# lab-emi/OpenDPD

Hardware: AMD Instinct MI355X
Metric: iq_samples_per_sec_train (higher is better)
Workload: dtype f32

## Files before the change

### opendpd_amd/csrc/capi.hip

```cpp
#include <dlfcn.h>

#include <mutex>
#include <set>
#include <utility>

#include "odpd_host.h"
#include "odpd_xchg.h"

using namespace odpd;

namespace {
enum Family { FAM_NONE = 0, FAM_GRU, FAM_LSTM, FAM_DELTA, FAM_JANET, FAM_TCNN, FAM_QAT, FAM_GMP, FAM_RVTDCNN, FAM_DVR, FAM_BOJ, FAM_APN, FAM_MCL, FAM_GRU2, FAM_QCELL };
inline Family family_of(int bb);
inline Family family_of(const odpd_model_t* m) {
    if (m->flags & ODPD_FLAG_QUANT_CELL) return FAM_QCELL;
    if (m->flags & ODPD_FLAG_TWO_LAYERS) return FAM_GRU2;
    if (m->bits_w > 0 && (m->backbone == ODPD_QGRU || m->backbone == ODPD_QGRU_AMP1 || m->backbone == ODPD_GRU || m->backbone == ODPD_DGRU ||
                          m->backbone == ODPD_TRES_DELTAGRU))
        return FAM_QAT;
    return family_of((int)m->backbone);
}
inline Family family_of(int bb) {
    switch (bb) {
    case ODPD_GRU: case ODPD_DGRU: case ODPD_QGRU: case ODPD_QGRU_AMP1: return FAM_GRU;
// ... 709 lines not shown
extern "C" int odpd_sweep_fwd_supported(const odpd_model_t* m, int B, int T) {
    return model_ok(m) && gru_family_model(m) && gru_sweep_eval_ok(m, B, T) ? 1 : 0;
}
extern "C" int odpd_sweep_s16_supported(const odpd_model_t* m) {
    return model_ok(m) && gru_family_model(m) && gru_s16_sweep_ok(m) ? 1 : 0;
}
extern "C" int64_t odpd_sweep_partial_rows(const odpd_model_t* m, int B, int T, int flags) {
    if (!model_ok(m) || B <= 0 || T <= 0 || !gru_family_model(m)) return ODPD_EUNSUPPORTED;
    if (flags & ODPD_SWEEP_S16) return gru_s16_sweep_ok(m) ? gru_s16_rows(m, B) : (int64_t)ODPD_EUNSUPPORTED;
    return gru_sweep_train_ok(m, B, T) ? gru_sweep_train_rows(m, B, T) : (int64_t)ODPD_EUNSUPPORTED;
}
extern "C" int64_t odpd_sweep_workspace_floats(const odpd_model_t* m, int B, int T, int flags) {
    if (!model_ok(m) || B <= 0 || T <= 0) return ODPD_EINVAL;
    if (init_state(m) || quant_cell(m)) return ODPD_EUNSUPPORTED;
    if (!(flags & ODPD_SWEEP_S16)) return 0;
    return odpd_sweep_s16_supported(m) ? gru_s16_ckpt_floats(m, B, T) : (int64_t)ODPD_EUNSUPPORTED;
}
extern "C" int odpd_train_epoch_sweep(void* stream, const odpd_model_t* m, int K, const odpd_sweep_run_t* runs, int loss_kind, const odpd_frames_t* fr,
                                      int batch, int64_t first_step, double beta1, double beta2, double eps, double weight_decay, double max_norm,
                                      int flags, void* scratch) {
    if (!model_ok(m) || K <= 0 || !runs || !epoch_frames_ok(fr, batch, false) || first_step <= 0 || !scratch) return ODPD_EINVAL;
    if (!sweep_runs_ok(K, runs, [](int) { return true; })) return ODPD_EINVAL;
    const int T = fr->frame_length;
    const bool s16 = (flags & ODPD_SWEEP_S16) != 0;
    if (!gru_family_model(m) || !frames_format_ok(m, fr)) return ODPD_EUNSUPPORTED;
    if (s16) {
        if (!gru_s16_sweep_ok(m)) return ODPD_EUNSUPPORTED;
        for (int k = 0; k < K; ++k)
            if (!runs[k].workspace) return ODPD_EINVAL;
    } else if (!epoch_shapes_served(fr, batch, 0, 1, [&](int B) { return gru_sweep_train_ok(m, B, T); })) {
        return ODPD_EUNSUPPORTED;
// ... 78 lines not shown
```

### opendpd_amd/csrc/gru_family.hip

```cpp
#include <algorithm>

#include "odpd_gru.h"

namespace odpd {

template <int R, int F, bool DG>
struct GruW {
    float wih[3][F];
    float b_r, b_z, b_in, b_hn;
    float wout[2], bout[2];
    float bhid;
    float woutf[2];
};

template <int R, int F, bool DG>
__device__ __forceinline__ void load_gru_w(GruW<R, F, DG>& w, const float* pl, const GruLayout& L, int row, int col) {
    const int H = L.H, o = 16 * row + col;
    const bool vo = o < H;
#pragma unroll
    for (int g = 0; g < 3; ++g)
#pragma unroll
        for (int i = 0; i < F; ++i) w.wih[g][i] = vo ? pl[L.o_w_ih + (g * H + o) * F + i] : 0.0f;
    w.b_r = vo ? pl[L.o_b_ih + o] + pl[L.o_b_hh + o] : 0.0f;
    w.b_z = vo ? pl[L.o_b_ih + H + o] + pl[L.o_b_hh + H + o] : 0.0f;
// ... 1330 lines not shown
        p.fwd_eval = eval || (knobs_free && B <= 8 && T >= 256) ? KS_EVAL : big;
        const bool bwd_gp = R == 1 && !s16 && knobs_free && (long)B <= (long)device_cus() * gp_blocks_per_cu(P, R, DG, T, false);
        p.bwd_w = bwd_gp ? KS_GP : big;
        p.bwd_dx = p.bwd_wdx = big;
        p.rot_rows = bwd_shape(R, ng).grid;
        p.bwd_rows = s16n ? gru_s16n_rows(m, B) : s16 ? gru_s16_bwd_rows(m, B) : bwd_gp ? std::max(gp_grid(P, R, DG, B, T), p.rot_rows) : p.rot_rows;
    }
    if (parts & GRU_PLAN_FUSED) {
        const int rot_grid = big == KS_ROT ? train_shape(P, R, DG, ng, T, nullptr).grid : 0;
        const bool too_long = R == 1 && rot_grid <= 0;
        if (big != KS_ROT) p.fused = big;
        else if (too_long) p.fused = KS_S16;
        else p.fused = gp_batch_fits(B, gp_blocks_per_cu(P, R, DG, T, false), 1) ? KS_GP : KS_ROT;
        switch (p.fused) {
        case KS_S16X: case KS_S16N: p.fused_rows = gru_s16n_rows(m, B); p.ws_floats = s16n_floats(); break;
        case KS_S16: p.fused_rows = gru_s16_rows(m, B); p.ws_floats = gru_s16_ckpt_floats(m, B, T); break;
        case KS_GP: p.fused_rows = gp_grid(P, R, DG, B, T); break;
        default: p.fused_rows = rot_grid > 0 ? rot_grid : ODPD_EUNSUPPORTED;
        }
    }
    if (parts & GRU_PLAN_LOSSDX) {
        const bool no_gain = R == 2 && !DG && m->hidden > 24 && tn.gp_max_batch < 0, knob_bars = tn.gp_max_batch >= 0 && B > tn.gp_max_batch;
        const int fz_grid = big == KS_ROT && !no_gain && !knob_bars ? gp_fz_grid(P, R, DG, B, T) : 0;
        p.lossdx = s16n ? (gru_s16x_ok(m) ? KS_S16X : KS_S16N) : s16 ? KS_S16 : fz_grid > 0 ? KS_GP : KS_ROT;
        switch (p.lossdx) {
        case KS_S16X: case KS_S16N: p.loss_rows = gru_s16n_rows(m, B); break;
        case KS_S16: p.loss_rows = gru_s16_rows(m, B); break;
        case KS_GP: p.loss_rows = fz_grid; break;
        default: {
            const int grid = train_shape(P, R, DG, ng, T, nullptr, true).grid;
            p.loss_rows = grid > 0 ? grid : ODPD_EUNSUPPORTED;
// ... 8 lines not shown
```

### opendpd_amd/csrc/gru_s16.hip

```cpp
#include "odpd_s16.h"

namespace odpd {

constexpr int kS16Groups = 15;
constexpr int kS16GroupsDx = 20;
template <int FM, bool DG, bool PACK = false>
__device__ __forceinline__ float4 s16_table_entry(const float* pl, const GruLayout& L, int grp, int m, int q) {
    const int H = L.H, OW = DG ? H + 6 : H;
    float v[4] = {0.f, 0.f, 0.f, 0.f};
#pragma unroll
    for (int e = 0; e < 4; ++e) {
        const int k = 4 * q + e;
        const bool mk = m < H && k < H;
        if (grp < 3) {
            v[e] = mk ? pl[L.o_w_hh + (grp * H + m) * H + k] * (grp < 2 ? kNegLog2e : 1.0f) : 0.0f;
            if (PACK && grp < 2 && k >= 13) v[e] = kNegLog2e * s16_wih_slot<FM, DG>(pl, L, grp, 1, m, k - 13);
        }
        else if (grp == 3) v[e] = kNegLog2e * s16_wih_slot<FM, DG>(pl, L, e >> 1, e & 1, m, q);
        else if (grp == 4) v[e] = e < 2 ? s16_wih_slot<FM, DG>(pl, L, 2, e, m, q) : 0.0f;
        else if (grp == 5) v[e] = k < H ? pl[L.o_b_hh + 2 * H + k] : 0.0f;
        else if (grp < 9) v[e] = mk ? pl[L.o_w_hh + ((grp - 6) * H + k) * H + m] : 0.0f;
        else if (grp == 9) v[e] = (DG && mk) ? pl[L.o_w_hid + m * H + k] : 0.0f;
        else if (grp == 10) v[e] = (DG && mk) ? pl[L.o_w_hid + k * H + m] : 0.0f;
        else if (grp == 11) v[e] = (DG && k < H) ? pl[L.o_b_hid + k] : 0.0f;
        else if (grp < 14) v[e] = k < H ? pl[L.o_w_out + (grp - 12) * OW + k] : 0.0f;
        else if (grp == 14) v[e] = s16_woutf_slot<FM, DG>(pl, L, e >> 1, e & 1, q);
        else if (grp < 18) v[e] = (m < S16Cfg<FM>::F && k < H) ? pl[L.o_w_ih + ((grp - 15) * H + k) * S16Cfg<FM>::F + m] : 0.0f;
        else v[e] = (DG && k < S16Cfg<FM>::F) ? pl[L.o_w_out + (grp - 18) * OW + H + k] : 0.0f;
    }
    return make_float4(v[0], v[1], v[2], v[3]);
}
template <int FM, bool DG, bool PACK = false>
__device__ __forceinline__ void s16_fill_table(float* tab, const float* pl, const GruLayout& L, int lane, int wave, int nwb,
                                               int ngroups = kS16Groups) {
    float4* t4 = reinterpret_cast<float4*>(tab);
    for (int grp = wave; grp < ngroups; grp += nwb)
        if (DG || (grp < 9 || grp > 11)) t4[grp * 64 + lane] = s16_table_entry<FM, DG, PACK>(pl, L, grp, lane & 15, lane >> 4);
    __syncthreads();
}

template <int FM>
struct S16Fw {
    float whh[3][4];
    float wih[3][2];
    f32x4 bhn;
};
template <int FM, bool DG>
struct S16Bw {
    float whhT[3][4];
    float whid[4], whidT[4];
    f32x4 bhid;
    f32x4 wout[2];
    float woutf[2][2];
};
// ... 67 lines not shown
        const f32x4 z4 = {0.f, 0.f, 0.f, 0.f};
#pragma unroll
        for (int g = 0; g < 3; ++g) { thh[g] = z4; tih[g] = z4; }
        thid = z4; db_hn = z4; db_hid = z4; dwout[0] = z4; dwout[1] = z4;
        dwf[0][0] = dwf[0][1] = dwf[1][0] = dwf[1][1] = 0.f;
#pragma unroll
        for (int j = 0; j < 4; ++j) vr[j] = vz[j] = 0.f;
    }
};
#ifdef ODPD_NO_PACKGRAD
constexpr bool s16_packgrad(bool pack, bool nw) { return false; }
#else
constexpr bool s16_packgrad(bool pack, bool nw) { return pack && nw; }
#endif

template <int FM, bool DG, bool FUSED, bool NW, bool DX, bool FULL, bool PACK = false>
__device__ __forceinline__ void s16_block(const SeqArgs& a, TabPtr tl, const float (&oh)[4], S16Grad<DG>& G,
                                          const float2* xs, const float2* ts, float2* dxs, float* tiles, int n, int q, int tloc,
                                          int nstep, bool valid, bool last_blk, f32x4 h, f32x4& dh, float (&hTn)[4],
                                          float& loss_acc) {
    constexpr int NCH = S16Cfg<FM>::NCH, S = kCkptStride;
    f32x4 hp_s[S], r_s[S], z_s[S], n_s[S], g_s[S];
    float fs_s[S][NCH];
    {
        S16Fw<FM> wf;
        s16_load_fw<FM>(wf, tl);
#pragma unroll
        for (int st = 0; st < S; ++st) {
            if (FULL || st < nstep) {
                const float2 xv = xs[n * kChunkPad + tloc + st];
                hp_s[st] = h;
                if constexpr (PACK) {
                    float pk[3];
                    s16_slots_pk<FM>(xv.x, xv.y, oh, fs_s[st], pk);
                    s16_cell_fwd<FM, true>(wf, fs_s[st], h, r_s[st], z_s[st], n_s[st], g_s[st], pk);
                } else {
// ... 13 lines not shown
        TabPtr tx = opaque(tl);
#pragma unroll
        for (int g = 0; g < 3; ++g) {
            const float4 v = tab_ld(tx, (15 + g) * 64);
            wihT[g][0] = v.x; wihT[g][1] = v.y; wihT[g][2] = v.z; wihT[g][3] = v.w;
        }
        wfD[0] = as_f32x4(tab_ld(tx, 18 * 64));
        wfD[1] = as_f32x4(tab_ld(tx, 19 * 64));
    }
    if (NW && DG && last_blk) {
        wave_lds_fence();
        tile_put(t_h, n, q, h);
        wave_lds_fence();
        tile_get(t_h, n, q, hTn);
    }
    const S16Loss lossc = s16_loss_setup(a.loss_kind == ODPD_LOSS_L2, valid ? a.inv_count : 0.0f, valid && q == 0);
#pragma unroll
    for (int st = S - 1; st >= 0; --st) {
        if (FULL || st < nstep) {
            __builtin_amdgcn_sched_barrier(0);
            const f32x4 hp = hp_s[st], r = r_s[st], z = z_s[st], nn = n_s[st], gh = g_s[st];
            f32x4 act, hid;
            const f32x4 ht = fma4(z, sub4(hp, nn), nn);
            if constexpr (DG) {
                hid = w.bhid;
#pragma unroll
                for (int c = 0; c < 4; ++c) hid = mfma4(w.whid[c], ht[c], hid);
                ODPD_EACH4 act[i] = relu_(hid[i]);
            } else {
                act = ht;
            }
// ... 1 lines not shown
            float dy0 = tv.x, dy1 = tv.y;
            if constexpr (FUSED) {
                float p0 = 0.0f, p1 = 0.0f;
#pragma unroll
                for (int c = 0; c < NCH; ++c) {
                    p0 = __builtin_fmaf(w.woutf[0][c], fs_s[st][c], p0);
                    p1 = __builtin_fmaf(w.woutf[1][c], fs_s[st][c], p1);
                }
#pragma unroll
                for (int e = 0; e < 4; ++e) {
                    p0 = __builtin_fmaf(w.wout[0][e], act[e], p0);
                    p1 = __builtin_fmaf(w.wout[1][e], act[e], p1);
                }
                const float y0 = quad_sum(p0), y1 = quad_sum(p1);
                const float d0 = y0 - tv.x, d1 = y1 - tv.y;
                s16_loss(lossc, d0, d1, dy0, dy1, loss_acc);
            }
            if constexpr (NW) {
#pragma unroll
                for (int c = 0; c < NCH; ++c) {
                    if (c < 2) {
                        G.dwf[0][c] = __builtin_fmaf(dy0, fs_s[st][c], G.dwf[0][c]);
                        G.dwf[1][c] = __builtin_fmaf(dy1, fs_s[st][c], G.dwf[1][c]);
                    }
                }
                G.dwout[0] = fma4(splat4(dy0), act, G.dwout[0]);
                G.dwout[1] = fma4(splat4(dy1), act, G.dwout[1]);
            }
            f32x4 dht, dhid;
            const f32x4 dact = fma4(splat4(dy0), w.wout[0], mul4(w.wout[1], splat4(dy1)));
            if constexpr (DG) {
// ... 163 lines not shown
        for (int c = 0; c < NCH; ++c) {
            const int k = 4 * c + q;
            const float v = row_sum16(G.dwf[cc][c < 2 ? c : 0]);
            if (n == 0) {
                if (DG && k < F) prow[L.o_w_out + cc * OW + H + k] = v;
                else if (k == F) prow[L.o_b_out + cc] = v;
            }
        }
    const float lp = row_sum16(loss_acc);
    if (n == 0 && q == 0) {
        prow[L.P] = lp;
        prow[L.P + 1] = 0.f; prow[L.P + 2] = 0.f; prow[L.P + 3] = 0.f;
    }
}

template <int FM, bool DG, int OCC, bool PACK, bool NW = true, bool DX = false>
__device__ __forceinline__ void gru16_train_body(const SeqArgs& a, const int bid, const int nbl) {
    constexpr int F = S16Cfg<FM>::F, NCH = S16Cfg<FM>::NCH, S = kCkptStride;
    constexpr int kGroups = DX ? kS16GroupsDx : kS16Groups;
    constexpr int kWave = (DX ? 3 : 2) * 2 * 16 * kChunkPad + (NW ? kS16Tiles * kTileFloats : 0) + kStageRowFloats;
    static_assert(NCH <= 2, "operand tables and dwf accumulators are sized for two K-chunks");
    extern __shared__ __attribute__((aligned(16))) float smem[];
    const int lane = threadIdx.x & 63, wave = threadIdx.x >> 6, nwb = blockDim.x >> 6;
    const int n = lane & 15, q = lane >> 4;
    const GruLayout L = gru_layout(a.H, F, DG);
    float* pl = smem;
    stage_params(pl, a.params, L.P);
    float* tab = smem + pad4(L.P);
    s16_fill_table<FM, DG, PACK>(tab, pl, L, lane, wave, nwb, kGroups);
    TabPtr tl = to_tab(reinterpret_cast<const float4*>(tab) + lane);
    float oh[4];
#pragma unroll
    for (int e = 0; e < 4; ++e) oh[e] = q == e ? 1.0f : 0.0f;
    float* wbase = tab + s16_tab_floats(kGroups) + (size_t)wave * kWave;
    float2* xs = reinterpret_cast<float2*>(wbase);
    float2* ts = xs + 16 * kChunkPad;
    float2* dxs = DX ? ts + 16 * kChunkPad : nullptr;
    float* tiles = reinterpret_cast<float*>(ts + (DX ? 2 : 1) * 16 * kChunkPad);
    unsigned long long* rows = reinterpret_cast<unsigned long long*>(wbase + kWave - kStageRowFloats);
    const bool bf16 = a.frames_bf16 != 0;
    const float2 kFillX = make_float2(0.5f, 0.5f), kFillT = make_float2(0.0f, 0.0f);
    if constexpr (NW)
        for (int i = lane; i < kTileFloats; i += 64) tiles[6 * kTileFloats + i] = 0.0f;
    S16Grad<DG> G;
    G.zero();
    float loss_acc = 0.0f;
    const int nwaves = nbl * nwb;
    for (int grp = bid * nwb + wave; grp < a.ngroups; grp += nwaves) {
        const int b0 = grp * 16;
        const bool valid = b0 + n < a.B;
        float4* ck = reinterpret_cast<float4*>(a.ckpt) + (size_t)grp * a.nck * 64 + lane;
        wave_lds_fence();
        stage_rows(rows, b0, a.B, a.T, lane, a.frame_idx, a.frame_stride);
        wave_lds_fence();
        {
            S16Fw<FM> w;
            s16_load_fw<FM>(w, tl);
            f32x4 h = {0.f, 0.f, 0.f, 0.f};
            for (int t0 = 0; t0 < a.T; t0 += kChunk) {
                const int len = min(kChunk, a.T - t0);
                StagedChunk<1> xc;
                stage_issue<1>(xc, {a.x}, rows, b0, a.B, t0, len, lane, {kFillX}, bf16);
                wave_lds_fence();
                stage_commit<1>(xc, {xs}, b0, a.B, len, lane, bf16);
                wave_lds_fence();
                int tt = 0;
                for (; tt + S <= len; tt += S) {
#pragma unroll
                    for (int i = 0; i < S; ++i) {
                        const float2 xv = xs[n * kChunkPad + tt + i];
                        float fs[NCH];
                        f32x4 r, z, nn, g;
                        if constexpr (PACK) {
                            float pk[3];
                            s16_slots_pk<FM>(xv.x, xv.y, oh, fs, pk);
                            s16_cell_fwd<FM, true>(w, fs, h, r, z, nn, g, pk);
                        } else {
                            s16_slots<FM>(xv.x, xv.y, oh, fs);
                            s16_cell_fwd<FM>(w, fs, h, r, z, nn, g);
                        }
                    }
                    const int t1 = t0 + tt + S;
                    if (t1 < a.T) ck[(size_t)(t1 / S) * 64] = make_float4(h[0], h[1], h[2], h[3]);
                }
                for (; tt < len; ++tt) {
                    const float2 xv = xs[n * kChunkPad + tt];
                    float fs[NCH];
                    f32x4 r, z, nn, g;
                    if constexpr (PACK) {
                        float pk[3];
                        s16_slots_pk<FM>(xv.x, xv.y, oh, fs, pk);
                        s16_cell_fwd<FM, true>(w, fs, h, r, z, nn, g, pk);
                    } else {
                        s16_slots<FM>(xv.x, xv.y, oh, fs);
                        s16_cell_fwd<FM>(w, fs, h, r, z, nn, g);
                    }
                }
            }
        }
        __builtin_amdgcn_fence(__ATOMIC_SEQ_CST, "workgroup");
        f32x4 dh = {0.f, 0.f, 0.f, 0.f};
        float hTn[4] = {0.f, 0.f, 0.f, 0.f};
        int cur_chunk = -1;
        float4 h0n = a.nck > 1 ? ck[(size_t)(a.nck - 1) * 64] : make_float4(0.f, 0.f, 0.f, 0.f);
        for (int blk = a.nck - 1; blk >= 0; --blk) {
            const int tb = blk * S, nstep = min(S, a.T - tb);
            const int chunk = tb / kChunk, t0 = chunk * kChunk;
            const f32x4 h0 = {h0n.x, h0n.y, h0n.z, h0n.w};
            h0n = blk > 1 ? ck[(size_t)(blk - 1) * 64] : make_float4(0.f, 0.f, 0.f, 0.f);
            if (chunk != cur_chunk) {
                if constexpr (DX) {
                    if (cur_chunk >= 0) {
                        const int pt0 = cur_chunk * kChunk;
                        wave_lds_fence();
                        stage_out<16>(dxs, a.dx, b0, a.B, a.T, pt0, min(kChunk, a.T - pt0), lane);
                    }
                }
                const int len = min(kChunk, a.T - t0);
                StagedChunk<2> xt;
                stage_issue<2>(xt, {a.x, a.target}, rows, b0, a.B, t0, len, lane, {kFillX, kFillT}, bf16);
                wave_lds_fence();
                stage_commit<2>(xt, {xs, ts}, b0, a.B, len, lane, bf16);
                wave_lds_fence();
                cur_chunk = chunk;
            }
            if (nstep == S)
                s16_block<FM, DG, true, NW, DX, true, PACK>(a, tl, oh, G, xs, ts, dxs, tiles, n, q, tb - t0, nstep, valid, blk == a.nck - 1, h0, dh, hTn, loss_acc);
            else
                s16_block<FM, DG, true, NW, DX, false, PACK>(a, tl, oh, G, xs, ts, dxs, tiles, n, q, tb - t0, nstep, valid, blk == a.nck - 1, h0, dh, hTn, loss_acc);
        }
        if constexpr (DX) {
            if (cur_chunk >= 0) {
                const int pt0 = cur_chunk * kChunk;
                wave_lds_fence();
                stage_out<16>(dxs, a.dx, b0, a.B, a.T, pt0, min(kChunk, a.T - pt0), lane);
                wave_lds_fence();
            }
        }
    }
    if constexpr (!NW) {
        const float lp = row_sum16(loss_acc);
        __syncthreads();
        if (lane == 0) smem[wave] = lp;
        __syncthreads();
// ... 4 lines not shown
            a.partials[(size_t)bid * kLossCols + threadIdx.x] = v;
        }
        return;
    }
    const int P4 = L.P + kLossCols;
    __syncthreads();
    s16_write_row<FM, DG, s16_packgrad(PACK, NW)>(smem + wave * P4, L, G, n, q, loss_acc);
    __syncthreads();
    float* prow = a.partials + (size_t)bid * P4;
    for (int i = threadIdx.x; i < P4; i += blockDim.x) {
        float v = smem[i];
        for (int wv = 1; wv < nwb; ++wv) v += smem[wv * P4 + i];
        prow[i] = v;
    }
}
template <int FM, bool DG, int OCC, bool PACK, bool NW = true, bool DX = false>
__global__ __launch_bounds__(64 * 4 * OCC, OCC) void gru16_train_kernel(SeqArgs a) {
    gru16_train_body<FM, DG, OCC, PACK, NW, DX>(a, blockIdx.x, gridDim.x);
}
template <int FM, bool DG, int OCC, bool PACK>
__global__ __launch_bounds__(64 * 4 * OCC, OCC) void gru16_train_sweep_kernel(SeqArgs a, const SweepRun* __restrict__ runs, int G, long long first) {
    const SweepRun r = runs[blockIdx.x / G];
    a.params = r.params; a.partials = r.partials; a.frame_idx = r.order + first; a.ckpt = r.workspace;
    gru16_train_body<FM, DG, OCC, PACK>(a, blockIdx.x % G, G);
}

__device__ __forceinline__ void s16_ckpt_store(float4* rec, int lane, int n, int q, int H, const f32x4& h) {
    const int nfull = H >> 2, rem = H & 3;
    if (q < nfull) rec[lane] = make_float4(h[0], h[1], h[2], h[3]);
    else if (q == nfull) {
        float* f = reinterpret_cast<float*>(rec + nfull * 16) + n;
        if (rem > 0) f[0] = h[0];
        if (rem > 1) f[16] = h[1];
        if (rem > 2) f[32] = h[2];
    }
}
__device__ __forceinline__ float4 s16_ckpt_load(const float4* rec, int lane, int n, int q, int H) {
    const int nfull = H >> 2, rem = H & 3;
    float4 v = make_float4(0.f, 0.f, 0.f, 0.f);
    if (q < nfull) v = rec[lane];
    else if (q == nfull) {
        const float* f = reinterpret_cast<const float*>(rec + nfull * 16) + n;
        if (rem > 0) v.x = f[0];
        if (rem > 1) v.y = f[16];
        if (rem > 2) v.z = f[32];
    }
    return v;
}

template <int FM, bool DG, bool PACK>
__global__ __launch_bounds__(1024) void gru16_fwd_kernel(SeqArgs a) {
    constexpr int F = S16Cfg<FM>::F, NCH = S16Cfg<FM>::NCH, S = kCkptStride;
    extern __shared__ __attribute__((aligned(16))) float smem[];
    const int lane = threadIdx.x & 63, wave = threadIdx.x >> 6, nwb = blockDim.x >> 6;
    const int n = lane & 15, q = lane >> 4;
    const GruLayout L = gru_layout(a.H, F, DG);
    float* pl = smem;
    stage_params(pl, a.params, L.P);
    float* tab = smem + pad4(L.P);
    s16_fill_table<FM, DG, PACK>(tab, pl, L, lane, wave, nwb);
    TabPtr tl = to_tab(reinterpret_cast<const float4*>(tab) + lane);
    float oh[4];
#pragma unroll
    for (int e = 0; e < 4; ++e) oh[e] = q == e ? 1.0f : 0.0f;
    float2* xs = reinterpret_cast<float2*>(tab + s16_tab_floats(kS16Groups)) + (size_t)wave * (2 * 16 * kChunkPad);
    float2* ys = xs + 16 * kChunkPad;
    S16Fw<FM> wf;
    s16_load_fw<FM>(wf, tl);
    S16Bw<FM, DG> wh;
    s16_load_bw<FM, DG>(wh, tl);
    const int nwaves = gridDim.x * nwb;
    for (int grp = blockIdx.x * nwb + wave; grp < a.ngroups; grp += nwaves) {
        const int b0 = grp * 16;
        float4* ck = a.ckpt ? reinterpret_cast<float4*>(a.ckpt) + (size_t)grp * a.nck * 64 : nullptr;
        f32x4 h = {0.f, 0.f, 0.f, 0.f};
        for (int t0 = 0; t0 < a.T; t0 += kChunk) {
            const int len = min(kChunk, a.T - t0);
            wave_lds_fence();
            stage_in<16>(xs, a.x, b0, a.B, a.T, t0, len, lane, make_float2(0.5f, 0.5f));
            wave_lds_fence();
            for (int tt = 0; tt < len; ++tt) {
                const float2 xv = xs[n * kChunkPad + tt];
                float fs[NCH];
                f32x4 r, z, nn, g, act;
                if constexpr (PACK) {
                    float pk[3];
                    s16_slots_pk<FM>(xv.x, xv.y, oh, fs, pk);
                    s16_cell_fwd<FM, true>(wf, fs, h, r, z, nn, g, pk);
                } else {
                    s16_slots<FM>(xv.x, xv.y, oh, fs);
                    s16_cell_fwd<FM>(wf, fs, h, r, z, nn, g);
                }
                if constexpr (DG) {
                    f32x4 hid = wh.bhid;
// ... 13 lines not shown
                for (int e = 0; e < 4; ++e) {
                    p0 = __builtin_fmaf(wh.wout[0][e], act[e], p0);
                    p1 = __builtin_fmaf(wh.wout[1][e], act[e], p1);
                }
                const float y0 = quad_sum(p0), y1 = quad_sum(p1);
                if (q == 0) ys[n * kChunkPad + tt] = make_float2(y0, y1);
                const int t1 = t0 + tt + 1;
                if (ck != nullptr && (t1 % S) == 0 && t1 < a.T) s16_ckpt_store(ck + (size_t)(t1 / S) * 64, lane, n, q, a.H, h);
            }
            wave_lds_fence();
            stage_out<16>(ys, a.y, b0, a.B, a.T, t0, len, lane);
        }
    }
}

template <int FM, bool DG, bool NW, bool DX, int WAVES, bool PACK = false>
__global__ __launch_bounds__(64 * WAVES, WAVES / 4) void gru16_bwd_kernel(SeqArgs a) {
    constexpr int F = S16Cfg<FM>::F, S = kCkptStride;
    constexpr int kGroups = DX ? kS16GroupsDx : kS16Groups;
    constexpr int kWave = (DX ? 3 : 2) * 2 * 16 * kChunkPad + (NW ? kS16Tiles * kTileFloats : 0);
    extern __shared__ __attribute__((aligned(16))) float smem[];
    const int lane = threadIdx.x & 63, wave = threadIdx.x >> 6, nwb = blockDim.x >> 6;
    const int n = lane & 15, q = lane >> 4;
    const GruLayout L = gru_layout(a.H, F, DG);
    float* pl = smem;
    stage_params(pl, a.params, L.P);
    float* tab = smem + pad4(L.P);
    s16_fill_table<FM, DG, PACK>(tab, pl, L, lane, wave, nwb, kGroups);
    TabPtr tl = to_tab(reinterpret_cast<const float4*>(tab) + lane);
    float oh[4];
#pragma unroll
    for (int e = 0; e < 4; ++e) oh[e] = q == e ? 1.0f : 0.0f;
    float* wbase = tab + s16_tab_floats(kGroups) + (size_t)wave * kWave;
    float2* xs = reinterpret_cast<float2*>(wbase);
    float2* dys = xs + 16 * kChunkPad;
    float2* dxs = DX ? dys + 16 * kChunkPad : nullptr;
    float* tiles = reinterpret_cast<float*>(dys + (DX ? 2 : 1) * 16 * kChunkPad);
    if constexpr (NW)
        for (int i = lane; i < kTileFloats; i += 64) tiles[6 * kTileFloats + i] = 0.0f;
    S16Grad<DG> G;
    G.zero();
    float unused = 0.0f;
    const int nwaves = gridDim.x * nwb;
    for (int grp = blockIdx.x * nwb + wave; grp < a.ngroups; grp += nwaves) {
        const int b0 = grp * 16;
        const float4* ck = reinterpret_cast<const float4*>(a.ckpt) + (size_t)grp * a.nck * 64;
        f32x4 dh = {0.f, 0.f, 0.f, 0.f};
        float hTn[4] = {0.f, 0.f, 0.f, 0.f};
        int cur_chunk = -1;
        float4 h0n = a.nck > 1 ? s16_ckpt_load(ck + (size_t)(a.nck - 1) * 64, lane, n, q, a.H) : make_float4(0.f, 0.f, 0.f, 0.f);
        for (int blk = a.nck - 1; blk >= 0; --blk) {
            const int tb = blk * S, nstep = min(S, a.T - tb);
            const int chunk = tb / kChunk, t0 = chunk * kChunk;
            const f32x4 h0 = {h0n.x, h0n.y, h0n.z, h0n.w};
            h0n = blk > 1 ? s16_ckpt_load(ck + (size_t)(blk - 1) * 64, lane, n, q, a.H) : make_float4(0.f, 0.f, 0.f, 0.f);
            if (chunk != cur_chunk) {
                if constexpr (DX) {
                    if (cur_chunk >= 0) {
                        const int pt0 = cur_chunk * kChunk;
                        wave_lds_fence();
                        stage_out<16>(dxs, a.dx, b0, a.B, a.T, pt0, min(kChunk, a.T - pt0), lane);
                    }
                }
                wave_lds_fence();
                const int len = min(kChunk, a.T - t0);
                stage_in<16>(xs, a.x, b0, a.B, a.T, t0, len, lane, make_float2(0.5f, 0.5f));
                stage_in<16>(dys, a.dy, b0, a.B, a.T, t0, len, lane, make_float2(0.0f, 0.0f));
                wave_lds_fence();
                cur_chunk = chunk;
            }
            if (nstep == S)
                s16_block<FM, DG, false, NW, DX, true, PACK>(a, tl, oh, G, xs, dys, dxs, tiles, n, q, tb - t0, nstep, true, blk == a.nck - 1, h0, dh, hTn, unused);
            else
                s16_block<FM, DG, false, NW, DX, false, PACK>(a, tl, oh, G, xs, dys, dxs, tiles, n, q, tb - t0, nstep, true, blk == a.nck - 1, h0, dh, hTn, unused);
        }
        if constexpr (DX) {
            if (cur_chunk >= 0) {
                const int pt0 = cur_chunk * kChunk;
                wave_lds_fence();
                stage_out<16>(dxs, a.dx, b0, a.B, a.T, pt0, min(kChunk, a.T - pt0), lane);
                wave_lds_fence();
            }
// ... 24 lines not shown
    return ngroups <= 4 * device_cus() ? 1 : 2;
}
static LaunchShape s16_shape(int ngroups) {
    LaunchShape ls;
    ls.waves = 4 * s16_occupancy(ngroups);
    const int need = (ngroups + ls.waves - 1) / ls.waves, cap = device_cus();
    ls.grid = need < cap ? need : cap;
    return ls;
}

int gru_s16_groups(int B) { return (B + 15) / 16; }
int64_t gru_s16_ckpt_floats(const odpd_model_t* m, int B, int T) {
    (void)m;
    return (int64_t)gru_s16_groups(B) * num_ckpt(T) * 256;
}
int gru_s16_rows(const odpd_model_t* m, int B) {
    (void)m;
    return s16_shape(gru_s16_groups(B)).grid;
}

template <int FM, typename F>
static int s16_occ_dispatch(const SeqArgs& a, F f) {
    if (s16_occupancy(a.ngroups) == 1) return f(int_c<1>{}, std::false_type{});
    if constexpr (S16Cfg<FM>::NCH == 2) { if (a.H <= 13) return f(int_c<2>{}, std::true_type{}); }
    return f(int_c<2>{}, std::false_type{});
}
template <typename F>
static int s16_feat_dispatch(int FM, F f) {
    switch (FM) {
    case FEAT_RAW2: return f(int_c<FEAT_RAW2>{}, std::false_type{});
    case FEAT_DGRU6: return f(int_c<FEAT_DGRU6>{}, std::true_type{});
    case FEAT_Q4: return f(int_c<FEAT_Q4>{}, std::false_type{});
    case FEAT_A4: return f(int_c<FEAT_A4>{}, std::false_type{});
    default: return ODPD_EUNSUPPORTED;
    }
}
template <int FM, bool DG>
static int launch_s16_occ(hipStream_t st, const SeqArgs& a, int P) {
    const LaunchShape ls = s16_shape(a.ngroups);
    return s16_occ_dispatch<FM>(a, [&](auto occ, auto pack) {
        return launch_lds(st, gru16_train_kernel<FM, DG, occ(), pack()>, ls.grid, 64 * ls.waves, s16_lds_bytes(P, ls.waves), a);
    });
}
template <int FM, bool DG>
static int launch_s16_lossdx_occ(hipStream_t st, const SeqArgs& a, int P) {
    const LaunchShape ls = s16_shape(a.ngroups);
    const size_t lds = ((size_t)pad4(P) + s16_tab_floats(kS16GroupsDx) + (size_t)ls.waves * (3 * 2 * 16 * kChunkPad + kStageRowFloats)) * sizeof(float);
    return s16_occ_dispatch<FM>(a, [&](auto occ, auto pack) {
        return launch_lds(st, gru16_train_kernel<FM, DG, occ(), pack(), false, true>, ls.grid, 64 * ls.waves, lds, a);
    });
}

static LaunchShape s16_fwd_shape(int ngroups) {
    LaunchShape ls;
    const int cus = device_cus();
    ls.waves = 4;
    while (ls.waves < 16 && ngroups > ls.waves * cus) ls.waves *= 2;
    const int need = (ngroups + ls.waves - 1) / ls.waves;
    ls.grid = need < cus ? need : cus;
    return ls;
}
static LaunchShape s16_bwd_shape(int ngroups, bool nw, bool dx) {
    LaunchShape ls;
    const int cus = device_cus();
    const int maxw = (nw && dx) ? 4 : 8;
    ls.waves = ngroups <= 4 * cus ? 4 : maxw;
    const int need = (ngroups + ls.waves - 1) / ls.waves;
    ls.grid = need < cus ? need : cus;
    return ls;
}
int gru_s16_bwd_rows(const odpd_model_t* m, int B) {
    (void)m;
    return s16_bwd_shape(gru_s16_groups(B), true, false).grid;
}

template <int FM, bool DG>
static int launch_s16_fwd(hipStream_t st, const SeqArgs& a, int P) {
    const LaunchShape ls = s16_fwd_shape(a.ngroups);
    const size_t lds = ((size_t)pad4(P) + s16_tab_floats(kS16Groups) + (size_t)ls.waves * 2 * 2 * 16 * kChunkPad) * sizeof(float);
    auto launch = [&](auto k) { return launch_lds(st, k, ls.grid, 64 * ls.waves, lds, a); };
    if constexpr (S16Cfg<FM>::NCH == 2) { if (a.H <= 13) return launch(gru16_fwd_kernel<FM, DG, true>); }
    return launch(gru16_fwd_kernel<FM, DG, false>);
}
template <int FM, bool DG, bool NW, bool DX, int WAVES>
static int launch_s16_bwd(hipStream_t st, const SeqArgs& a, int P) {
    LaunchShape ls = s16_bwd_shape(a.ngroups, NW, DX);
    if (NW) ls.grid = s16_bwd_shape(a.ngroups, true, false).grid;
    const int waves = ls.waves < WAVES ? ls.waves : WAVES;
    const int wave_floats = (DX ? 3 : 2) * 2 * 16 * kChunkPad + (NW ? kS16Tiles * kTileFloats : 0);
    size_t lds = ((size_t)pad4(P) + s16_tab_floats(DX ? kS16GroupsDx : kS16Groups) + (size_t)waves * wave_floats) * sizeof(float);
    if (NW && lds < reduce_scratch_bytes(P, waves)) lds = reduce_scratch_bytes(P, waves);
    auto launch = [&](auto k) { return launch_lds(st, k, ls.grid, 64 * waves, lds, a); };
    if constexpr (S16Cfg<FM>::NCH == 2 && NW && !DX) { if (a.H <= 13) return launch(gru16_bwd_kernel<FM, DG, NW, DX, WAVES, true>); }
    return launch(gru16_bwd_kernel<FM, DG, NW, DX, WAVES>);
}
template <int FM, bool DG>
static int launch_s16_bwd_mode(hipStream_t st, const SeqArgs& a, int P) {
    return s16_bwd_dispatch(a, [&](auto nw, auto dx) { return launch_s16_bwd<FM, DG, nw(), dx(), (nw() && dx()) ? 4 : 8>(st, a, P); });
}

int gru_s16_fwd(hipStream_t st, const odpd_model_t* m, const SeqArgs& a0) {
    int FM; bool DG;
    if (!gru_cfg(m, FM, DG) || m->hidden > 16) return ODPD_EUNSUPPORTED;
    SeqArgs a = a0;
// ... 12 lines not shown

int gru_s16_lossdx(hipStream_t st, const odpd_model_t* m, const SeqArgs& a0) {
    int FM; bool DG;
    if (!gru_cfg(m, FM, DG) || m->hidden > 16) return ODPD_EUNSUPPORTED;
    if (!a0.ckpt || !a0.dx || !a0.partials || !a0.target) return ODPD_EINVAL;
    SeqArgs a = a0;
    a.ngroups = gru_s16_groups(a.B);
    const int P = gru_param_count(m->hidden, FM, DG);
    return s16_feat_dispatch(FM, [&](auto fm, auto dg) { return launch_s16_lossdx_occ<fm(), dg()>(st, a, P); });
}

template <int FM, bool DG>
static int launch_s16_sweep_occ(hipStream_t st, const SeqArgs& a, int P, const SweepRun* runs, int K, long long first) {
    const LaunchShape ls = s16_shape(a.ngroups);
    return s16_occ_dispatch<FM>(a, [&](auto occ, auto pack) {
        return launch_lds(st, gru16_train_sweep_kernel<FM, DG, occ(), pack()>, ls.grid * K, 64 * ls.waves, s16_lds_bytes(P, ls.waves), a, runs, ls.grid, first);
    });
}
bool gru_s16_sweep_ok(const odpd_model_t* m) {
    int FM; bool DG;
    return gru_cfg(m, FM, DG) && m->hidden <= 16 && m->bits_w == 0 && !(m->flags & ODPD_FLAG_TWO_LAYERS);
}
int gru_s16_sweep_train(hipStream_t st, const odpd_model_t* m, const SeqArgs& a0, const SweepRun* runs, int K, long long first) {
    int FM; bool DG;
    if (!gru_cfg(m, FM, DG) || !gru_s16_sweep_ok(m) || K <= 0 || !runs) return ODPD_EUNSUPPORTED;
    SeqArgs a = a0;
    a.ngroups = gru_s16_groups(a.B);
    const int P = gru_param_count(m->hidden, FM, DG);
    return s16_feat_dispatch(FM, [&](auto fm, auto dg) { return launch_s16_sweep_occ<fm(), dg()>(st, a, P, runs, K, first); });
}

int gru_s16_train(hipStream_t st, const odpd_model_t* m, const SeqArgs& a0) {
    int FM; bool DG;
    if (!gru_cfg(m, FM, DG) || m->hidden > 16) return ODPD_EUNSUPPORTED;
    if (!a0.ckpt) return ODPD_EINVAL;
    SeqArgs a = a0;
    a.ngroups = gru_s16_groups(a.B);
    const int P = gru_param_count(m->hidden, FM, DG);
    return s16_feat_dispatch(FM, [&](auto fm, auto dg) { return launch_s16_occ<fm(), dg()>(st, a, P); });
}

}
```

### opendpd_amd/csrc/odpd_host.h

```cpp
#pragma once
#include <hip/hip_runtime.h>
#include <stdint.h>
#include <string.h>

#include <type_traits>

#include "../../include/opendpd_hip.h"
#include "odpd_device.h"

namespace odpd {

#define ODPD_CHECK_HIP(expr)                         \
    do {                                             \
        hipError_t _e = (expr);                      \
        if (_e != hipSuccess) return (int)_e;        \
    } while (0)

constexpr int kLossCols = 4;

inline int rows_per_seq(int H) { return H <= 16 ? 1 : (H <= 32 ? 2 : 0); }
inline int seqs_per_wave(int R) { return 4 / R; }
inline int num_groups(int B, int R) { int spw = seqs_per_wave(R); return (B + spw - 1) / spw; }
__host__ __device__ inline int num_ckpt_hd(int T) { return (T + kCkptStride - 1) / kCkptStride; }
inline int num_ckpt(int T) { return num_ckpt_hd(T); }
// ... 316 lines not shown
int64_t gru_s16n_ckpt_floats(const odpd_model_t* m, int B, int T);
bool gru_s16x_ok(const odpd_model_t* m);
int gru_s16x_lossdx(hipStream_t s, const odpd_model_t* m, const SeqArgs& a, int grid);
int64_t gru_s16x_ckpt_floats(const odpd_model_t* m, int B, int T);
bool gru_s16x_train_ok(const odpd_model_t* m);
int gru_s16x_train(hipStream_t s, const odpd_model_t* m, const SeqArgs& a, int grid);
int gru_s16x_fwd(hipStream_t s, const odpd_model_t* m, const SeqArgs& a);
int gru_s16x_bwd(hipStream_t s, const odpd_model_t* m, const SeqArgs& a, int rows);
int launch_clip_adamw(hipStream_t st, int64_t P, float* params, float* grad, float* exp_avg, float* exp_avg_sq, int64_t step,
                      double lr, double beta1, double beta2, double eps, double weight_decay, double max_norm, float* norm_out,
                      float* loss_out, float inv_count, const unsigned char* skip = nullptr, const XchgDev* xchg = nullptr);
int launch_clip_optim(hipStream_t st, int kind, int64_t P, float* params, float* grad, float* state1, float* state2, int64_t step, double lr,
                      double max_norm, float* norm_out, float* loss_out, float inv_count, const unsigned char* skip = nullptr,
                      const XchgDev* xchg = nullptr);
int64_t gru_s16_ckpt_floats(const odpd_model_t* m, int B, int T);
int delta_gp_train(hipStream_t s, const odpd_model_t* m, const SeqArgs& a);
int lstm_family_fwd(hipStream_t s, const odpd_model_t* m, const SeqArgs& a);
int lstm_family_bwd(hipStream_t s, const odpd_model_t* m, const SeqArgs& a);
bool lstm_train_uses_s16(const odpd_model_t* m, int B);
int lstm_gp_train(hipStream_t s, const odpd_model_t* m, const SeqArgs& a);
int lstm_s16_train(hipStream_t s, const odpd_model_t* m, const SeqArgs& a);
int lstm_s16_rows(const odpd_model_t* m, int B);
int64_t lstm_s16_workspace_floats(const odpd_model_t* m, int B, int T);
int delta_family_fwd(hipStream_t s, const odpd_model_t* m, const SeqArgs& a);
int delta_family_bwd(hipStream_t s, const odpd_model_t* m, const SeqArgs& a);
bool delta_uses_s16(const odpd_model_t* m, int B);
int delta_s16_launch(hipStream_t s, const odpd_model_t* m, const SeqArgs& a, int mode);
int delta_s16_rows(const odpd_model_t* m, int B);
int64_t delta_s16_ckpt_floats(const odpd_model_t* m, int B, int T);
struct JanetLayout { int H, o_wa, o_ba, o_wp1, o_bp1, o_wp2, o_bp2, o_wf, o_bf, o_wg, o_bg, o_wo, o_bo, P; };
// ... 94 lines not shown
```

### opendpd_amd/csrc/odpd_s16.h

```cpp
#pragma once
#include "odpd_seq.h"

namespace odpd {

constexpr int kTilePitch = 20;
constexpr int kTileFloats = 16 * kTilePitch;
constexpr int kS16Tiles = 7;
constexpr int kS16WaveFloats = 2 * 2 * 16 * kChunkPad + kS16Tiles * kTileFloats;

template <int FM> struct S16Cfg {
    static constexpr int F = FeatDim<FM>::F;
    static constexpr int NCH = (F + 4) / 4;
};

__host__ __device__ constexpr int s16_tab_floats(int groups) { return groups * 64 * 4; }

template <int FM, bool DG>
__device__ __forceinline__ float s16_wih_slot(const float* pl, const GruLayout& L, int g, int c, int m, int q) {
    constexpr int F = S16Cfg<FM>::F, NCH = S16Cfg<FM>::NCH;
    const int H = L.H, k = 4 * c + q;
    if (c >= NCH || m >= H) return 0.0f;
    if (k < F) return pl[L.o_w_ih + (g * H + m) * F + k];
    if (k == F) return pl[L.o_b_ih + g * H + m] + (g < 2 ? pl[L.o_b_hh + g * H + m] : 0.0f);
    return 0.0f;
// ... 127 lines not shown
struct S16Loss { float c2, c1, w2, w1; };
__device__ __forceinline__ S16Loss s16_loss_setup(bool l2, float sc, bool counts) {
    S16Loss L;
    L.c2 = l2 ? 2.0f * sc : 0.0f; L.c1 = l2 ? 0.0f : sc;
    L.w2 = (l2 && counts) ? 1.0f : 0.0f; L.w1 = (!l2 && counts) ? 1.0f : 0.0f;
    return L;
}
__device__ __forceinline__ float s16_sign(float d) {
    return __builtin_copysignf(__builtin_amdgcn_fmed3f(__builtin_fabsf(d) * 0x1p100f, 0.0f, 1.0f), d);
}
__device__ __forceinline__ void s16_loss(const S16Loss& L, float d0, float d1, float& dy0, float& dy1, float& acc) {
    dy0 = __builtin_fmaf(L.c1, s16_sign(d0), L.c2 * d0);
    dy1 = __builtin_fmaf(L.c1, s16_sign(d1), L.c2 * d1);
    acc = __builtin_fmaf(L.w2, __builtin_fmaf(d0, d0, d1 * d1), acc);
    acc = __builtin_fmaf(L.w1, __builtin_fabsf(d0) + __builtin_fabsf(d1), acc);
}
__device__ __forceinline__ float relu_gate(float v) { return __builtin_amdgcn_fmed3f(v * 0x1p100f, 0.0f, 1.0f); }

__device__ __forceinline__ float quad_sum(float v) {
#ifdef ODPD_QUAD_SUM_LDS
    v += swap16(v);
    v += __shfl_xor(v, 32);
    return v;
#else
    const int iv = __builtin_bit_cast(int, v);
    const auto a = __builtin_amdgcn_permlane16_swap(iv, iv, false, false);
    const int a0 = a[0], a1 = a[1];
    const float s = __builtin_bit_cast(float, a0) + __builtin_bit_cast(float, a1);
    const int is = __builtin_bit_cast(int, s);
    const auto b = __builtin_amdgcn_permlane32_swap(is, is, false, false);
// ... 38 lines not shown
```

Before: 8.690 billion.

## Skip redundant tail forward, add L2-specialised loss, decouple S16 block size

The fused S16 train kernel now runs its forward pass only up to the last checkpoint instead of the full sequence, since the backward pass recomputes the final block anyway. It also adds a compile-time L2 loss specialisation that drops the L1 sign path, and makes the recompute block size a separate compile-time knob with its own workspace sizing. The standalone forward and backward kernels switch from synchronous stage_in to the row-staged issue/commit loader, and their LDS budgets grow to hold the row table. More template instantiations raise code size, and the workspace size must stay consistent with the new block count.

```diff
diff --git a/opendpd_amd/csrc/capi.hip b/opendpd_amd/csrc/capi.hip
--- a/opendpd_amd/csrc/capi.hip
+++ b/opendpd_amd/csrc/capi.hip
@@ -747,7 +747,7 @@
     if (!model_ok(m) || B <= 0 || T <= 0) return ODPD_EINVAL;
     if (init_state(m) || quant_cell(m)) return ODPD_EUNSUPPORTED;
     if (!(flags & ODPD_SWEEP_S16)) return 0;
-    return odpd_sweep_s16_supported(m) ? gru_s16_ckpt_floats(m, B, T) : (int64_t)ODPD_EUNSUPPORTED;
+    return odpd_sweep_s16_supported(m) ? gru_s16_train_ws_floats(m, B, T) : (int64_t)ODPD_EUNSUPPORTED;
 }
 extern "C" int odpd_train_epoch_sweep(void* stream, const odpd_model_t* m, int K, const odpd_sweep_run_t* runs, int loss_kind, const odpd_frames_t* fr,
                                       int batch, int64_t first_step, double beta1, double beta2, double eps, double weight_decay, double max_norm,
diff --git a/opendpd_amd/csrc/gru_family.hip b/opendpd_amd/csrc/gru_family.hip
--- a/opendpd_amd/csrc/gru_family.hip
+++ b/opendpd_amd/csrc/gru_family.hip
@@ -1368,7 +1368,7 @@
         else p.fused = gp_batch_fits(B, gp_blocks_per_cu(P, R, DG, T, false), 1) ? KS_GP : KS_ROT;
         switch (p.fused) {
         case KS_S16X: case KS_S16N: p.fused_rows = gru_s16n_rows(m, B); p.ws_floats = s16n_floats(); break;
-        case KS_S16: p.fused_rows = gru_s16_rows(m, B); p.ws_floats = gru_s16_ckpt_floats(m, B, T); break;
+        case KS_S16: p.fused_rows = gru_s16_rows(m, B); p.ws_floats = gru_s16_train_ws_floats(m, B, T); break;
         case KS_GP: p.fused_rows = gp_grid(P, R, DG, B, T); break;
         default: p.fused_rows = rot_grid > 0 ? rot_grid : ODPD_EUNSUPPORTED;
         }
diff --git a/opendpd_amd/csrc/gru_s16.hip b/opendpd_amd/csrc/gru_s16.hip
--- a/opendpd_amd/csrc/gru_s16.hip
+++ b/opendpd_amd/csrc/gru_s16.hip
@@ -38,6 +38,12 @@
         if (DG || (grp < 9 || grp > 11)) t4[grp * 64 + lane] = s16_table_entry<FM, DG, PACK>(pl, L, grp, lane & 15, lane >> 4);
     __syncthreads();
 }
+
+#ifndef ODPD_S16_BLOCK
+#define ODPD_S16_BLOCK kCkptStride
+#endif
+constexpr int kS16Block = ODPD_S16_BLOCK;
+static_assert(kS16Block >= 1 && kChunk % kS16Block == 0, "a block never straddles two staged chunks");
 
 template <int FM>
 struct S16Fw {
@@ -135,12 +141,12 @@
 constexpr bool s16_packgrad(bool pack, bool nw) { return pack && nw; }
 #endif
 
-template <int FM, bool DG, bool FUSED, bool NW, bool DX, bool FULL, bool PACK = false>
+template <int FM, bool DG, bool FUSED, bool NW, bool DX, bool FULL, bool PACK = false, int S = kCkptStride, bool L2C = false>
 __device__ __forceinline__ void s16_block(const SeqArgs& a, TabPtr tl, const float (&oh)[4], S16Grad<DG>& G,
                                           const float2* xs, const float2* ts, float2* dxs, float* tiles, int n, int q, int tloc,
                                           int nstep, bool valid, bool last_blk, f32x4 h, f32x4& dh, float (&hTn)[4],
                                           float& loss_acc) {
-    constexpr int NCH = S16Cfg<FM>::NCH, S = kCkptStride;
+    constexpr int NCH = S16Cfg<FM>::NCH;
     f32x4 hp_s[S], r_s[S], z_s[S], n_s[S], g_s[S];
     float fs_s[S][NCH];
     {
@@ -184,7 +190,7 @@
         wave_lds_fence();
         tile_get(t_h, n, q, hTn);
     }
-    const S16Loss lossc = s16_loss_setup(a.loss_kind == ODPD_LOSS_L2, valid ? a.inv_count : 0.0f, valid && q == 0);
+    const S16Loss lossc = s16_loss_setup(L2C || a.loss_kind == ODPD_LOSS_L2, valid ? a.inv_count : 0.0f, valid && q == 0);
 #pragma unroll
     for (int st = S - 1; st >= 0; --st) {
         if (FULL || st < nstep) {
@@ -216,7 +222,8 @@
                 }
                 const float y0 = quad_sum(p0), y1 = quad_sum(p1);
                 const float d0 = y0 - tv.x, d1 = y1 - tv.y;
-                s16_loss(lossc, d0, d1, dy0, dy1, loss_acc);
+                if constexpr (L2C) s16_loss_l2(lossc, d0, d1, dy0, dy1, loss_acc);
+                else s16_loss(lossc, d0, d1, dy0, dy1, loss_acc);
             }
             if constexpr (NW) {
 #pragma unroll
@@ -410,9 +417,9 @@
     }
 }
 
-template <int FM, bool DG, int OCC, bool PACK, bool NW = true, bool DX = false>
+template <int FM, bool DG, int OCC, bool PACK, bool NW = true, bool DX = false, bool L2C = false>
 __device__ __forceinline__ void gru16_train_body(const SeqArgs& a, const int bid, const int nbl) {
-    constexpr int F = S16Cfg<FM>::F, NCH = S16Cfg<FM>::NCH, S = kCkptStride;
+    constexpr int F = S16Cfg<FM>::F, NCH = S16Cfg<FM>::NCH, S = NW ? kS16Block : kCkptStride;
     constexpr int kGroups = DX ? kS16GroupsDx : kS16Groups;
     constexpr int kWave = (DX ? 3 : 2) * 2 * 16 * kChunkPad + (NW ? kS16Tiles * kTileFloats : 0) + kStageRowFloats;
     static_assert(NCH <= 2, "operand tables and dwf accumulators are sized for two K-chunks");
@@ -441,6 +448,11 @@
     S16Grad<DG> G;
     G.zero();
     float loss_acc = 0.0f;
+#ifdef ODPD_S16_FULL_FWD
+    const int Tf = a.T;
+#else
+    const int Tf = (a.nck - 1) * S;
+#endif
     const int nwaves = nbl * nwb;
     for (int grp = bid * nwb + wave; grp < a.ngroups; grp += nwaves) {
         const int b0 = grp * 16;
@@ -453,8 +465,8 @@
             S16Fw<FM> w;
             s16_load_fw<FM>(w, tl);
             f32x4 h = {0.f, 0.f, 0.f, 0.f};
-            for (int t0 = 0; t0 < a.T; t0 += kChunk) {
-                const int len = min(kChunk, a.T - t0);
+            for (int t0 = 0; t0 < Tf; t0 += kChunk) {
+                const int len = min(kChunk, Tf - t0);
                 StagedChunk<1> xc;
                 stage_issue<1>(xc, {a.x}, rows, b0, a.B, t0, len, lane, {kFillX}, bf16);
                 wave_lds_fence();
@@ -479,6 +491,7 @@
                     const int t1 = t0 + tt + S;
                     if (t1 < a.T) ck[(size_t)(t1 / S) * 64] = make_float4(h[0], h[1], h[2], h[3]);
                 }
+#ifdef ODPD_S16_FULL_FWD
                 for (; tt < len; ++tt) {
                     const float2 xv = xs[n * kChunkPad + tt];
                     float fs[NCH];
@@ -492,6 +505,7 @@
                         s16_cell_fwd<FM>(w, fs, h, r, z, nn, g);
                     }
                 }
+#endif
             }
         }
         __builtin_amdgcn_fence(__ATOMIC_SEQ_CST, "workgroup");
@@ -521,9 +535,9 @@
                 cur_chunk = chunk;
             }
             if (nstep == S)
-                s16_block<FM, DG, true, NW, DX, true, PACK>(a, tl, oh, G, xs, ts, dxs, tiles, n, q, tb - t0, nstep, valid, blk == a.nck - 1, h0, dh, hTn, loss_acc);
+                s16_block<FM, DG, true, NW, DX, true, PACK, S, L2C>(a, tl, oh, G, xs, ts, dxs, tiles, n, q, tb - t0, nstep, valid, blk == a.nck - 1, h0, dh, hTn, loss_acc);
             else
-                s16_block<FM, DG, true, NW, DX, false, PACK>(a, tl, oh, G, xs, ts, dxs, tiles, n, q, tb - t0, nstep, valid, blk == a.nck - 1, h0, dh, hTn, loss_acc);
+                s16_block<FM, DG, true, NW, DX, false, PACK, S, L2C>(a, tl, oh, G, xs, ts, dxs, tiles, n, q, tb - t0, nstep, valid, blk == a.nck - 1, h0, dh, hTn, loss_acc);
         }
         if constexpr (DX) {
             if (cur_chunk >= 0) {
@@ -558,15 +572,15 @@
         prow[i] = v;
     }
 }
-template <int FM, bool DG, int OCC, bool PACK, bool NW = true, bool DX = false>
+template <int FM, bool DG, int OCC, bool PACK, bool NW = true, bool DX = false, bool L2C = false>
 __global__ __launch_bounds__(64 * 4 * OCC, OCC) void gru16_train_kernel(SeqArgs a) {
-    gru16_train_body<FM, DG, OCC, PACK, NW, DX>(a, blockIdx.x, gridDim.x);
-}
-template <int FM, bool DG, int OCC, bool PACK>
+    gru16_train_body<FM, DG, OCC, PACK, NW, DX, L2C>(a, blockIdx.x, gridDim.x);
+}
+template <int FM, bool DG, int OCC, bool PACK, bool L2C>
 __global__ __launch_bounds__(64 * 4 * OCC, OCC) void gru16_train_sweep_kernel(SeqArgs a, const SweepRun* __restrict__ runs, int G, long long first) {
     const SweepRun r = runs[blockIdx.x / G];
     a.params = r.params; a.partials = r.partials; a.frame_idx = r.order + first; a.ckpt = r.workspace;
-    gru16_train_body<FM, DG, OCC, PACK>(a, blockIdx.x % G, G);
+    gru16_train_body<FM, DG, OCC, PACK, true, false, L2C>(a, blockIdx.x % G, G);
 }
 
 __device__ __forceinline__ void s16_ckpt_store(float4* rec, int lane, int n, int q, int H, const f32x4& h) {
@@ -592,6 +606,7 @@
     return v;
 }
 
+constexpr int kS16FwdWaveFloats = 2 * 2 * 16 * kChunkPad + kStageRowFloats;
 template <int FM, bool DG, bool PACK>
 __global__ __launch_bounds__(1024) void gru16_fwd_kernel(SeqArgs a) {
     constexpr int F = S16Cfg<FM>::F, NCH = S16Cfg<FM>::NCH, S = kCkptStride;
@@ -607,8 +622,10 @@
     float oh[4];
 #pragma unroll
     for (int e = 0; e < 4; ++e) oh[e] = q == e ? 1.0f : 0.0f;
-    float2* xs = reinterpret_cast<float2*>(tab + s16_tab_floats(kS16Groups)) + (size_t)wave * (2 * 16 * kChunkPad);
+    float* wbase = tab + s16_tab_floats(kS16Groups) + (size_t)wave * kS16FwdWaveFloats;
+    float2* xs = reinterpret_cast<float2*>(wbase);
     float2* ys = xs + 16 * kChunkPad;
+    unsigned long long* rows = reinterpret_cast<unsigned long long*>(wbase + kS16FwdWaveFloats - kStageRowFloats);
     S16Fw<FM> wf;
     s16_load_fw<FM>(wf, tl);
     S16Bw<FM, DG> wh;
@@ -618,10 +635,15 @@
         const int b0 = grp * 16;
         float4* ck = a.ckpt ? reinterpret_cast<float4*>(a.ckpt) + (size_t)grp * a.nck * 64 : nullptr;
         f32x4 h = {0.f, 0.f, 0.f, 0.f};
+        wave_lds_fence();
+        stage_rows(rows, b0, a.B, a.T, lane, nullptr, 0);
+        wave_lds_fence();
         for (int t0 = 0; t0 < a.T; t0 += kChunk) {
             const int len = min(kChunk, a.T - t0);
+            StagedChunk<1> xc;
+            stage_issue<1>(xc, {a.x}, rows, b0, a.B, t0, len, lane, {make_float2(0.5f, 0.5f)}, false);
             wave_lds_fence();
-            stage_in<16>(xs, a.x, b0, a.B, a.T, t0, len, lane, make_float2(0.5f, 0.5f));
+            stage_commit<1>(xc, {xs}, b0, a.B, len, lane, false);
             wave_lds_fence();
             for (int tt = 0; tt < len; ++tt) {
                 const float2 xv = xs[n * kChunkPad + tt];
@@ -665,11 +687,14 @@
     }
 }
 
+__host__ __device__ constexpr int s16_bwd_wave_floats(bool nw, bool dx) {
+    return (dx ? 3 : 2) * 2 * 16 * kChunkPad + (nw ? kS16Tiles * kTileFloats : 0) + kStageRowFloats;
+}
 template <int FM, bool DG, bool NW, bool DX, int WAVES, bool PACK = false>
 __global__ __launch_bounds__(64 * WAVES, WAVES / 4) void gru16_bwd_kernel(SeqArgs a) {
     constexpr int F = S16Cfg<FM>::F, S = kCkptStride;
     constexpr int kGroups = DX ? kS16GroupsDx : kS16Groups;
-    constexpr int kWave = (DX ? 3 : 2) * 2 * 16 * kChunkPad + (NW ? kS16Tiles * kTileFloats : 0);
+    constexpr int kWave = s16_bwd_wave_floats(NW, DX);
     extern __shared__ __attribute__((aligned(16))) float smem[];
     const int lane = threadIdx.x & 63, wave = threadIdx.x >> 6, nwb = blockDim.x >> 6;
     const int n = lane & 15, q = lane >> 4;
@@ -687,6 +712,7 @@
     float2* dys = xs + 16 * kChunkPad;
     float2* dxs = DX ? dys + 16 * kChunkPad : nullptr;
     float* tiles = reinterpret_cast<float*>(dys + (DX ? 2 : 1) * 16 * kChunkPad);
+    unsigned long long* rows = reinterpret_cast<unsigned long long*>(wbase + kWave - kStageRowFloats);
     if constexpr (NW)
         for (int i = lane; i < kTileFloats; i += 64) tiles[6 * kTileFloats + i] = 0.0f;
     S16Grad<DG> G;
@@ -696,6 +722,9 @@
     for (int grp = blockIdx.x * nwb + wave; grp < a.ngroups; grp += nwaves) {
         const int b0 = grp * 16;
         const float4* ck = reinterpret_cast<const float4*>(a.ckpt) + (size_t)grp * a.nck * 64;
+        wave_lds_fence();
+        stage_rows(rows, b0, a.B, a.T, lane, nullptr, 0);
+        wave_lds_fence();
         f32x4 dh = {0.f, 0.f, 0.f, 0.f};
         float hTn[4] = {0.f, 0.f, 0.f, 0.f};
         int cur_chunk = -1;
@@ -713,10 +742,11 @@
                         stage_out<16>(dxs, a.dx, b0, a.B, a.T, pt0, min(kChunk, a.T - pt0), lane);
                     }
                 }
-                wave_lds_fence();
                 const int len = min(kChunk, a.T - t0);
-                stage_in<16>(xs, a.x, b0, a.B, a.T, t0, len, lane, make_float2(0.5f, 0.5f));
-                stage_in<16>(dys, a.dy, b0, a.B, a.T, t0, len, lane, make_float2(0.0f, 0.0f));
+                StagedChunk<2> xd;
+                stage_issue<2>(xd, {a.x, a.dy}, rows, b0, a.B, t0, len, lane, {make_float2(0.5f, 0.5f), make_float2(0.0f, 0.0f)}, false);
+                wave_lds_fence();
+                stage_commit<2>(xd, {xs, dys}, b0, a.B, len, lane, false);
                 wave_lds_fence();
                 cur_chunk = chunk;
             }
@@ -771,6 +801,11 @@
     (void)m;
     return (int64_t)gru_s16_groups(B) * num_ckpt(T) * 256;
 }
+static int s16_train_nck(int T) { return (T + kS16Block - 1) / kS16Block; }
+int64_t gru_s16_train_ws_floats(const odpd_model_t* m, int B, int T) {
+    (void)m;
+    return (int64_t)gru_s16_groups(B) * s16_train_nck(T) * 256;
+}
 int gru_s16_rows(const odpd_model_t* m, int B) {
     (void)m;
     return s16_shape(gru_s16_groups(B)).grid;
@@ -781,6 +816,13 @@
     if (s16_occupancy(a.ngroups) == 1) return f(int_c<1>{}, std::false_type{});
     if constexpr (S16Cfg<FM>::NCH == 2) { if (a.H <= 13) return f(int_c<2>{}, std::true_type{}); }
     return f(int_c<2>{}, std::false_type{});
+}
+template <typename F>
+static int s16_loss_dispatch(const SeqArgs& a, F f) {
+#ifndef ODPD_S16_NO_L2C
+    if (a.loss_kind == ODPD_LOSS_L2) return f(std::true_type{});
+#endif
+    return f(std::false_type{});
 }
 template <typename F>
 static int s16_feat_dispatch(int FM, F f) {
@@ -796,7 +838,9 @@
 static int launch_s16_occ(hipStream_t st, const SeqArgs& a, int P) {
     const LaunchShape ls = s16_shape(a.ngroups);
     return s16_occ_dispatch<FM>(a, [&](auto occ, auto pack) {
-        return launch_lds(st, gru16_train_kernel<FM, DG, occ(), pack()>, ls.grid, 64 * ls.waves, s16_lds_bytes(P, ls.waves), a);
+        return s16_loss_dispatch(a, [&](auto l2) {
+            return launch_lds(st, gru16_train_kernel<FM, DG, occ(), pack(), true, false, l2()>, ls.grid, 64 * ls.waves, s16_lds_bytes(P, ls.waves), a);
+        });
     });
 }
 template <int FM, bool DG>
@@ -804,7 +848,9 @@
     const LaunchShape ls = s16_shape(a.ngroups);
     const size_t lds = ((size_t)pad4(P) + s16_tab_floats(kS16GroupsDx) + (size_t)ls.waves * (3 * 2 * 16 * kChunkPad + kStageRowFloats)) * sizeof(float);
     return s16_occ_dispatch<FM>(a, [&](auto occ, auto pack) {
-        return launch_lds(st, gru16_train_kernel<FM, DG, occ(), pack(), false, true>, ls.grid, 64 * ls.waves, lds, a);
+        return s16_loss_dispatch(a, [&](auto l2) {
+            return launch_lds(st, gru16_train_kernel<FM, DG, occ(), pack(), false, true, l2()>, ls.grid, 64 * ls.waves, lds, a);
+        });
     });
 }
 
@@ -834,7 +880,7 @@
 template <int FM, bool DG>
 static int launch_s16_fwd(hipStream_t st, const SeqArgs& a, int P) {
     const LaunchShape ls = s16_fwd_shape(a.ngroups);
-    const size_t lds = ((size_t)pad4(P) + s16_tab_floats(kS16Groups) + (size_t)ls.waves * 2 * 2 * 16 * kChunkPad) * sizeof(float);
+    const size_t lds = ((size_t)pad4(P) + s16_tab_floats(kS16Groups) + (size_t)ls.waves * kS16FwdWaveFloats) * sizeof(float);
     auto launch = [&](auto k) { return launch_lds(st, k, ls.grid, 64 * ls.waves, lds, a); };
     if constexpr (S16Cfg<FM>::NCH == 2) { if (a.H <= 13) return launch(gru16_fwd_kernel<FM, DG, true>); }
     return launch(gru16_fwd_kernel<FM, DG, false>);
@@ -844,7 +890,7 @@
     LaunchShape ls = s16_bwd_shape(a.ngroups, NW, DX);
     if (NW) ls.grid = s16_bwd_shape(a.ngroups, true, false).grid;
     const int waves = ls.waves < WAVES ? ls.waves : WAVES;
-    const int wave_floats = (DX ? 3 : 2) * 2 * 16 * kChunkPad + (NW ? kS16Tiles * kTileFloats : 0);
+    const int wave_floats = s16_bwd_wave_floats(NW, DX);
     size_t lds = ((size_t)pad4(P) + s16_tab_floats(DX ? kS16GroupsDx : kS16Groups) + (size_t)waves * wave_floats) * sizeof(float);
     if (NW && lds < reduce_scratch_bytes(P, waves)) lds = reduce_scratch_bytes(P, waves);
     auto launch = [&](auto k) { return launch_lds(st, k, ls.grid, 64 * waves, lds, a); };
@@ -887,7 +933,10 @@
 static int launch_s16_sweep_occ(hipStream_t st, const SeqArgs& a, int P, const SweepRun* runs, int K, long long first) {
     const LaunchShape ls = s16_shape(a.ngroups);
     return s16_occ_dispatch<FM>(a, [&](auto occ, auto pack) {
-        return launch_lds(st, gru16_train_sweep_kernel<FM, DG, occ(), pack()>, ls.grid * K, 64 * ls.waves, s16_lds_bytes(P, ls.waves), a, runs, ls.grid, first);
+        return s16_loss_dispatch(a, [&](auto l2) {
+            return launch_lds(st, gru16_train_sweep_kernel<FM, DG, occ(), pack(), l2()>, ls.grid * K, 64 * ls.waves, s16_lds_bytes(P, ls.waves), a, runs,
+                              ls.grid, first);
+        });
     });
 }
 bool gru_s16_sweep_ok(const odpd_model_t* m) {
@@ -899,6 +948,7 @@
     if (!gru_cfg(m, FM, DG) || !gru_s16_sweep_ok(m) || K <= 0 || !runs) return ODPD_EUNSUPPORTED;
     SeqArgs a = a0;
     a.ngroups = gru_s16_groups(a.B);
+    a.nck = s16_train_nck(a.T);
     const int P = gru_param_count(m->hidden, FM, DG);
     return s16_feat_dispatch(FM, [&](auto fm, auto dg) { return launch_s16_sweep_occ<fm(), dg()>(st, a, P, runs, K, first); });
 }
@@ -909,6 +959,7 @@
     if (!a0.ckpt) return ODPD_EINVAL;
     SeqArgs a = a0;
     a.ngroups = gru_s16_groups(a.B);
+    a.nck = s16_train_nck(a.T);
     const int P = gru_param_count(m->hidden, FM, DG);
     return s16_feat_dispatch(FM, [&](auto fm, auto dg) { return launch_s16_occ<fm(), dg()>(st, a, P); });
 }
diff --git a/opendpd_amd/csrc/odpd_host.h b/opendpd_amd/csrc/odpd_host.h
--- a/opendpd_amd/csrc/odpd_host.h
+++ b/opendpd_amd/csrc/odpd_host.h
@@ -354,6 +354,7 @@
                       double max_norm, float* norm_out, float* loss_out, float inv_count, const unsigned char* skip = nullptr,
                       const XchgDev* xchg = nullptr);
 int64_t gru_s16_ckpt_floats(const odpd_model_t* m, int B, int T);
+int64_t gru_s16_train_ws_floats(const odpd_model_t* m, int B, int T);
 int delta_gp_train(hipStream_t s, const odpd_model_t* m, const SeqArgs& a);
 int lstm_family_fwd(hipStream_t s, const odpd_model_t* m, const SeqArgs& a);
 int lstm_family_bwd(hipStream_t s, const odpd_model_t* m, const SeqArgs& a);
diff --git a/opendpd_amd/csrc/odpd_s16.h b/opendpd_amd/csrc/odpd_s16.h
--- a/opendpd_amd/csrc/odpd_s16.h
+++ b/opendpd_amd/csrc/odpd_s16.h
@@ -165,6 +165,11 @@
     dy1 = __builtin_fmaf(L.c1, s16_sign(d1), L.c2 * d1);
     acc = __builtin_fmaf(L.w2, __builtin_fmaf(d0, d0, d1 * d1), acc);
     acc = __builtin_fmaf(L.w1, __builtin_fabsf(d0) + __builtin_fabsf(d1), acc);
+}
+__device__ __forceinline__ void s16_loss_l2(const S16Loss& L, float d0, float d1, float& dy0, float& dy1, float& acc) {
+    dy0 = L.c2 * d0;
+    dy1 = L.c2 * d1;
+    acc = __builtin_fmaf(L.w2, __builtin_fmaf(d0, d0, d1 * d1), acc);
 }
 __device__ __forceinline__ float relu_gate(float v) { return __builtin_amdgcn_fmed3f(v * 0x1p100f, 0.0f, 1.0f); }
 
```

Measured after the change: 8.800 billion (median of 6 runs). +1.3%, better.
